# kuboyoo/alphazero-general-ori

Measured on AMD Instinct MI355X. Metric: self-play rollouts/sec (32k boards, 2p Splendor) at 1/2/4/8 MI355X, higher is better.
Workload: dtype fp32 (network) / int8 (boards) / f64 (tree statistics)

## Files before the change

alphazero-general-ori_amd/csrc/mcts.hip:

```cpp
#include <hip/hip_runtime.h>

#include <cmath>
#include <cstring>
#include <new>

#include "../../include/splendor_amd.h"

#include "board_phases.h"
#include "mcts_device.h"
#include "nn_stage.h"
#include "spl_ctx.h"

using namespace spl;

#ifndef SPL_BOUNDS_CHECK
#define SPL_BOUNDS_CHECK 0
#endif
#if SPL_BOUNDS_CHECK
__device__ unsigned long long g_bounds[4 + 64];
__device__ __noinline__ void bounds_note(int site, long long v, int t) {
    atomicAdd(&g_bounds[4 + (site & 63)], 1ull);
    if (atomicAdd(&g_bounds[0], 1ull) == 0) {
        g_bounds[1] = (unsigned long long)v; g_bounds[2] = (unsigned long long)site; g_bounds[3] = (unsigned long long)t;
    }
// ... 504 lines not shown
constexpr int GC_WG_MAX_PROBE = 1024;
__device__ unsigned long long g_gc_probe[GC_WG_MAX_PROBE][16];
__device__ unsigned long long g_gc_probe_max[GC_WG_MAX_PROBE][8];
#define GPROBE(k)                                                                 \
    if (threadIdx.x == 0) {                                                       \
        const uint64_t c_ = __builtin_readcyclecounter();                         \
        gacc[k] += c_ - glast;                                                    \
        glast = c_;                                                               \
    }
#else
#define GPROBE(k)
#endif
constexpr int GC_NOFIT = -2;
#ifndef GC_SR
#define GC_SR 8
#endif
#ifndef GC_CR
#define GC_CR 4
#endif
template <int CR = 4>
__device__ int compact_tree(const Pools &P, int t, int root, int root_round, const GcScr &S, GcLds &L,
                            int bunits, bool linked = false) {
    const int tid = threadIdx.x;
    TreeHdr *H = P.hdr + t;
    const int nc = H->node_count;
    const int rootl = root >= 0 ? node_l(P, root) : -1;
    int32_t *remap = S.remap;
#if GC_PROBE
    uint64_t gacc[8] = {0, 0, 0, 0, 0, 0, 0, 0}, glast = __builtin_readcyclecounter();
    const uint64_t gstart = glast;
#endif
    if (linked) {
        if (tid < 64) mark_linked(P, t, rootl, remap, S.queue);
        __syncthreads();
    }
    int kept = 0;
    for (int base = 0; base < nc; base += GCT) {
        const int i = base + tid;
        bool keep = false;
        if (i < nc) keep = i == rootl || (linked ? remap[i] == 1 : P.nd[node_g(P, t, i)].h.round > root_round);
        int tot;
        const int ex = block_scan(keep ? 1 : 0, tot, L);
        if (i < nc) remap[i] = keep ? kept + ex : -1;
        kept += tot;
    }
    __syncthreads();
    GPROBE(0)
    for (int i = tid; i < nc; i += GCT) {
        int sz = -1;
        if (remap[i] >= 0) {
            sz = 0;
            const int g = node_g(P, t, i);
            const Node nd = P.nd[g];
            if (!nd.h.term) sz = nd.c.ec + REC_UNITS * nd.c.vcnt();
        }
        S.nvs[i] = sz;
    }
    __syncthreads();
    if (tid < 64) {
        const int l = tid;
        int run = 0;
        constexpr int PD = 4;
        int pre[PD];
#pragma unroll
        for (int d = 0; d < PD; d++) pre[d] = 64 * d + l < nc ? S.nvs[64 * d + l] : -1;
        for (int base = 0; base < nc; base += 64) {
            const int i = base + l;
            const int szk = pre[0];
#pragma unroll
            for (int d = 0; d + 1 < PD; d++) pre[d] = pre[d + 1];
            pre[PD - 1] = base + 64 * PD + l < nc ? S.nvs[base + 64 * PD + l] : -1;
            const bool kept = szk >= 0;
            const int sz = kept ? szk : 0;
            bool pending = sz > 0;
            int start = run;
            for (;;) {
                const int x = pending ? sz : 0;
                int incl = x;
#pragma unroll
                for (int o = 1; o < 64; o <<= 1) {
                    const int y = __shfl_up(incl, o, 64);
                    if (l >= o) incl += y;
                }
                const int st = run + incl - x;
                const bool strad = pending && (st & (UPG - 1)) + sz > UPG;
                const uint64_t m = __ballot(strad);
                if (!m) {
                    if (pending) start = st;
                    run += __shfl(incl, 63, 64);
                    break;
                }
                const int f = __ffsll((unsigned long long)m) - 1;
                if (pending && l < f) { start = st; pending = false; }
                run = (__builtin_amdgcn_readlane(st, f) & ~(UPG - 1)) + UPG;
            }
            if (kept) S.nvs[i] = start;
        }
        if (l == 0) L.bc[0] = run;
    }
    __syncthreads();
    const int run = L.bc[0];
    GPROBE(1)
    if (run > H->epg * UPG) return GC_NOFIT;
    __syncthreads();
    int my_units = 0;
    for (int base = 0; base < nc; base += GCT) {
        const int i = base + tid;
        const int ni = i < nc ? remap[i] : -1;
        uint64_t k0 = 0, k1 = 0;
        Node nd{};
        int vs = 0;
        if (ni >= 0) {
            const int g = node_g(P, t, i);
            k0 = P.nkey0[g]; k1 = P.nkey1[g];
            nd = P.nd[g];
            vs = S.nvs[i];
        }
        __syncthreads();
        if (ni >= 0) {
            const int ng = node_g(P, t, ni);
            const bool term = nd.h.term;
            const int ec = nd.c.ec, vcnt = term ? 0 : nd.c.vcnt();
            const int sz = term ? 0 : ec + REC_UNITS * vcnt;
            Node w = nd;
            S.queue[ni] = term ? -1 : nd.h.bchild;
            S.ost[ni] = nd.c.eb(); S.ovb[ni] = nd.c.vb(); S.oec[ni] = term ? 0 : ec;
            if (!term) {
                w.c.set_eb(ec > 0 ? unit_g(P, t, vs) : 0, vcnt);
                w.c.set_vb(vcnt > 0 ? unit_g(P, t, vs + ec) : 0, vcnt);
            }
            w.h.h2 = -1; w.h.h3 = -1;
            P.nkey0[ng] = k0; P.nkey1[ng] = k1;
            P.nd[ng] = w;
            S.cs[ni] = vs; S.cnt[ni] = sz; S.inv[ni] = i;
            my_units += sz;
        }
    }
    int units;
    (void)block_scan(my_units, units, L);
    GPROBE(2)
    for (int ni = tid; ni < kept; ni += GCT) {
        const int ch = S.queue[ni];
        if (ch >= 0) {
            BCHK(IN_TREE(P, t, ch, nc), 56, ((long long)ni << 32) | (uint32_t)ch, t, (void)0);
            const int nl = remap[node_l(P, ch)];
            P.nd[node_g(P, t, ni)].h.bchild = nl >= 0 ? node_g(P, t, nl) : -1;
            BCHK(nl < 0 || P.nd[node_g(P, t, nl)].h.round == P.nd[node_g(P, t, ni)].h.round + 1, 40,
                 ((long long)ni << 32) | (uint32_t)nl, t, (void)0);
        }
    }
    for (int k = tid; k < run; k += GCT) S.own[k] = -1;
    __syncthreads();
    for (int ni = tid; ni < kept; ni += GCT) {
        const int c0 = S.cs[ni], c = S.cnt[ni];
        for (int e = 0; e < c; e++) S.own[c0 + e] = ni;
    }
    __syncthreads();
    GPROBE(3)
    constexpr int SR = GC_SR;
    for (int k0 = 0; k0 < run; k0 += GCT * SR) {
        int j[SR];
#pragma unroll
        for (int r = 0; r < SR; r++) {
            const int k = k0 + GCT * r + tid;
            j[r] = k < run ? S.own[k] : -1;
        }
        int64_t src[SR];
        bool link[SR];
#pragma unroll
        for (int r = 0; r < SR; r++) {
            src[r] = 0; link[r] = false;
            if (j[r] >= 0) {
                const int rel = k0 + GCT * r + tid - S.cs[j[r]], ec = S.oec[j[r]];
                if (rel < ec) {
                    src[r] = S.ost[j[r]] + rel;
                } else {
                    const int rr = rel - ec;
                    src[r] = S.ovb[j[r]] + rr;
                    link[r] = rr % REC_UNITS == REC_LINK_UNIT;
                }
            }
        }
        uint64_t v[SR];
#pragma unroll
        for (int r = 0; r < SR; r++) v[r] = j[r] >= 0 ? P.eu[src[r]] : 0;
#pragma unroll
// ... 470 lines not shown
            for (int k = 0; k < 7; k++) P.out_valid[slot * 7 + k] = P.ex_valid[x * 7 + k];
#pragma unroll
            for (int i = 0; i < 4; i++) {
                const int src = (i + px) % N;
                P.out_winner[slot * 4 + i] = i < N ? r[src < N ? src : 0] : 0.f;
                P.out_scdiff[slot * 4 + i] = i < N ? f[src < N ? src : 0] - f[px < N ? px : 0] : 0;
                P.out_q[slot * 4 + i] = P.ex_q[x * 4 + i];
            }
            P.out_meta[slot * 4 + 0] = (int)gb;
            P.out_meta[slot * 4 + 1] = gno;
            P.out_meta[slot * 4 + 2] = j;
            P.out_meta[slot * 4 + 3] = px;
            P.flq[fq0 + j] = make_int2((int)x, (int)slot);
        }
        __threadfence_block();
        __builtin_amdgcn_wave_barrier();
        if (l == 0) H->games_done += 1;
        deal_game<N>(P, C, t, b, ub[w]);
        nxt = 0;
    } else if (l == 0) {
        H->player = nxt;
        H->episode_step = step;
    }
    __threadfence_block();
    __builtin_amdgcn_wave_barrier();
    wave_store_board<N>(P.board + (size_t)t * Lx::S, b);
    wave_roll_players<N>(s, b, nxt);
    begin_search<N>(P, C, t, s, !ended, false);
    const int nroot = uniform(H->root);
    if (nroot >= 0 && uniform(H->noise_pending) && !uniform(H->gc_queued)) {
        const Node nd0 = P.nd[nroot];
        NodeRun r = run_of(nd0.c);
        r.eb = (int64_t)uniform64((uint64_t)r.eb); r.vb = (int64_t)uniform64((uint64_t)r.vb);
        r.ec = uniform(r.ec);
        const int cand = noise_kept_root(P, C, t, r, ST_DIR | (uint32_t)uniform(H->move_no), pbits[w],
                                         reinterpret_cast<float *>(pterm[w]), pprior[w], pact[w],
                                         reinterpret_cast<int16_t *>(pcnt[w]),
                                         reinterpret_cast<double *>(pprior[w]), (int)(sizeof(pprior[w]) / 8));
        wave_lds_fence();
        int ca;
        float cp, np;
        wave_cand(P, r.eb, r.ec, cand, ca, cp, np);
        const bool forced = uniform(H->forced) != 0;
        Pick pk{-1, 0, -1, 0};
        if (!forced) pk = scan_run(P, r, nd0.h.ns, nd0.h.qs, C.cpuct, C.fpu, false, 0);
        if (l == 0) {
            H->noise_pending = 0;
            Node w2 = nd0;
            w2.c.cand = (int16_t)cand; w2.c.ca = (int16_t)ca; w2.c.cp = cp; w2.c.np = np;
            w2.h.set_pick(pk.e, pk.a, pk.e >= 0 && pk.child >= 0 ? P.nd[pk.child].h.term : 0);
            w2.h.bchild = pk.e >= 0 ? pk.child : -1;
            w2.h.h2 = -1; w2.h.h3 = -1;
            w2.h.bvi = pk.e >= 0 ? P.ep(r.eb + pk.e)->vi : (int16_t)-1;
            P.nd[nroot] = w2;
        }
    }
}

__device__ __forceinline__ void grid_copy(void *dst, const void *src, size_t bytes) {
    const size_t tid = (size_t)blockIdx.x * blockDim.x + threadIdx.x, nth = (size_t)gridDim.x * blockDim.x;
    if (((uintptr_t)dst | (uintptr_t)src) % 16 == 0) {
        const size_t nv = bytes / 16;
        uint4 *d = (uint4 *)dst;
        const uint4 *s = (const uint4 *)src;
        for (size_t i = tid; i < nv; i += nth) d[i] = s[i];
        for (size_t i = nv * 16 + tid; i < bytes; i += nth) ((uint8_t *)dst)[i] = ((const uint8_t *)src)[i];
    } else {
        for (size_t i = tid; i < bytes; i += nth) ((uint8_t *)dst)[i] = ((const uint8_t *)src)[i];
    }
}

__global__ void k_drain_copy(Pools P, int S, int max, int8_t *st, float *pi, uint64_t *valid,
                             float *winner, int32_t *scdiff, float *q, int32_t *meta, int n) {
    const int k = min(P.counters[0], min(max, P.out_cap));
    if (pi) grid_copy(pi, P.out_pi, (size_t)k * SPL_ACTIONS * 4);
    if (st) grid_copy(st, P.out_state, (size_t)k * S);
    if (valid) grid_copy(valid, P.out_valid, (size_t)k * 7 * 8);
    if (meta) grid_copy(meta, P.out_meta, (size_t)k * 4 * 4);
    const size_t tid = (size_t)blockIdx.x * blockDim.x + threadIdx.x, nth = (size_t)gridDim.x * blockDim.x;
    for (size_t i = tid; i < (size_t)k * n; i += nth) {
        const size_t e = i / (size_t)n, j = i - e * (size_t)n;
        if (winner) winner[i] = P.out_winner[e * 4 + j];
        if (scdiff) scdiff[i] = P.out_scdiff[e * 4 + j];
        if (q) q[i] = P.out_q[e * 4 + j];
    }
}

__global__ void k_drain_reset(Pools P, int max, int32_t *n_out) {
    const int c = P.counters[0];
    const int k = min(c, min(max, P.out_cap));
    if (n_out) *n_out = k;
    P.counters[1] += min(c, P.out_cap) - k;
    P.counters[0] = 0;
}

__device__ __forceinline__ void term_values(const Pools &P, int g, float v[4]) {
    const float4 e = *reinterpret_cast<const float4 *>(&P.nd[g].c);
    v[0] = e.x; v[1] = e.y; v[2] = e.z; v[3] = e.w;
}
__device__ __forceinline__ Node term_node(const float v[4], int rd) {
    Node n{};
    n.h.bchild = -1; n.h.h2 = -1; n.h.h3 = -1; n.h.set_pick(-1, 0, 0); n.h.ns = 0;
    n.h.term = 1; n.h.round = (uint8_t)rd; n.h.qs = 0.0;
    *reinterpret_cast<float4 *>(&n.c) = make_float4(v[0], v[1], v[2], v[3]);
    n.h.bvi = -1;
    n.c.ec = 0; n.c.cand = 0; n.c.ca = 0; n.c.pad = 0; n.c.cp = 0.f; n.c.np = -1.f;
    return n;
// ... 27 lines not shown
    uint64_t a = 0, b = 0;
    for (int i = 0; i < Lay<N>::ROWS; i++) {
        const uint64_t x = row(s, i) | ((uint64_t)i << 56);
        a ^= mix64(x ^ 0x243F6A8885A308D3ull);
        b ^= mix64(x ^ 0x13198A2E03707344ull);
    }
    k0 = a;
    k1 = b | 1ull;
}
template <int N>
__device__ __forceinline__ void lane_tree_step(int8_t *s, int a) {
    Chance ch{nullptr, 0, 0, 0, 0};
    int nxt;
    switch (move_kind_of(a)) {
        case MK_GEMS: nxt = make_move<N, MK_GEMS>(s, a, 0, true, ch); break;
        case MK_BUY: nxt = make_move<N, MK_BUY>(s, a, 0, true, ch); break;
        case MK_RESERVE: nxt = make_move<N, MK_RESERVE>(s, a, 0, true, ch); break;
        default: nxt = make_move<N, MK_BUY_RESERVED>(s, a, 0, true, ch); break;
    }
    if (nxt) lane_roll_players<N>(s, nxt);
}

#ifndef SELECT_PROBE
#define SELECT_PROBE 0
#endif
#if SELECT_PROBE
__device__ unsigned long long g_sel_probe[16];
#define SPROBE(k)                                                  \
    {                                                              \
        const uint64_t c_ = __builtin_readcyclecounter();          \
        pacc[k] += c_ - plast;                                     \
        plast = c_;                                                \
    }
#else
#define SPROBE(k)
#endif
#ifndef PATH_CHUNK
#define PATH_CHUNK 8
#endif
enum { LS_DESCEND = 0, LS_EXPAND = 1, LS_DONE = 2 };

#ifndef SELECT_ASM
#define SELECT_ASM 1
#endif
#define SEL_STORES 2
#define SEL_W_OWN 3
#define SEL_W_HINT 8
#define SEL_W_HINT1 9
static_assert(SEL_W_OWN == 1 + SEL_STORES, "own child load: behind SC + the stores");
static_assert(SEL_W_HINT == SEL_STORES + 2 * (1 + SEL_STORES) && SEL_W_HINT1 == SEL_W_HINT + 1,
              "hinted record: two levels back");
#define SEL_STR2(x) #x
#define SEL_STR(x) SEL_STR2(x)
#define SEL_BODY(SA, SC, K)                                                                     \
    "v_cmp_le_i32 vcc, 0, v240\n"                       \
    "v_cmp_le_i32 %[T], 0, v243\n"                      \
    "s_and_b64 vcc, vcc, %[T]\n"                                                               \
    "v_cmp_gt_i32 %[T], %[pcap], v233\n"                \
    "s_and_b64 vcc, vcc, %[T]\n"                                                               \
    "s_and_b64 exec, exec, vcc\n"                                                              \
    "s_cbranch_execz L_done_%=\n"                                                              \
    "v_cmp_ne_u32 vcc, v240, v234\n"                  \
    "s_and_saveexec_b64 %[SV], vcc\n"                   \
    "s_mov_b64 %[INV], exec\n"                                                                 \
    "s_cbranch_execz L_nf" K "_%=\n"                                                           \
    "v_mad_u64_u32 v[238:239], %[CC], v240, 64, %[nd]\n"                                       \
    "global_load_dwordx4 " SA ", v[238:239], off\n"                                            \
    "L_nf" K "_%=:\n"                                                                          \
    "s_mov_b64 exec, %[SV]\n"                                                                  \
    "v_cmp_gt_u32 vcc, %[lim], v242\n"                  \
    "v_cndmask_b32 v226, v240, v242, vcc\n"             \
    "v_mad_u64_u32 v[238:239], %[CC], v226, 64, %[nd]\n"                                       \
    "global_load_dwordx4 " SC ", v[238:239], off\n"                                            \
    "v_mad_u64_u32 v[238:239], %[CC], v233, 4, v[252:253]\n"         \
    "global_store_dword v[238:239], v232, off\n"                                               \
    "v_and_b32 v236, 0xffff, v243\n"                                \
    "v_bfe_u32 v237, v243, 16, 15\n"                                                           \
    "v_lshl_or_b32 v236, v237, 9, v236\n"                                                      \
    "v_mad_u64_u32 v[238:239], %[CC], v233, 4, v[254:255]\n"                                   \
    "global_store_dword v[238:239], v236, off\n"                                               \
    "v_add_u32 v233, 1, v233\n"                                                                \
    "v_mov_b32 v232, v240\n"                                                                   \
    "v_mov_b32 v234, v235\n"                       \
    "v_mov_b32 v235, v226\n"                                                                   \
    "s_cmp_eq_u64 %[INV], 0\n"                                                                 \
    "s_cbranch_scc1 L_av" K "_%=\n"                                                            \
    "s_waitcnt vmcnt(" SEL_STR(SEL_W_OWN) ")\n"          \
    "s_mov_b32 %[F], 1\n"                                                                      \
    "s_branch L_sel" K "_%=\n"                                                                 \
    "L_av" K "_%=:\n"                                   \
    "s_cmp_eq_u32 %[F], 0\n"                            \
    "s_cbranch_scc1 L_a8" K "_%=\n"                     \
    "s_waitcnt vmcnt(" SEL_STR(SEL_W_HINT1) ")\n"                                              \
    "s_branch L_a0" K "_%=\n"                                                                  \
    "L_a8" K "_%=:\n"                                                                          \
    "s_waitcnt vmcnt(" SEL_STR(SEL_W_HINT) ")\n"                                               \
    "L_a0" K "_%=:\n"                                                                          \
    "s_mov_b32 %[F], 0\n"                                                                      \
    "L_sel" K "_%=:\n"
#define SEL_TAKE(R)                                                                             \
    "v_mov_b32 v240, v" #R "\n"                                                                \
    "v_mov_b32 v241, v" #R "+1\n"
__device__ __forceinline__ void descend_linked_asm(int &node, int &depth, NodeLink &rec, const Node *nd, int pcap,
                                                   int32_t *path_n, int32_t *path_x, uint64_t runm, int lim) {
    int r0 = rec.bchild, r1 = rec.h2, r2 = rec.h3;
    int r3 = (int)((uint32_t)(uint16_t)rec.best | ((uint32_t)rec.babt << 16));
    uint64_t T, SV, INV, CC, SAVE;
    int F;
    asm volatile(
        "s_mov_b64 %[SAVE], exec\n"
        "s_mov_b32 %[F], 1\n"
        "v_mov_b32 v232, %[node]\n"
        "v_mov_b32 v233, %[depth]\n"
        "v_mov_b32 v240, %[r0]\n"
        "v_mov_b32 v241, %[r1]\n"
        "v_mov_b32 v242, %[r2]\n"
        "v_mov_b32 v243, %[r3]\n"
        "v_mov_b32 v234, -1\n"
        "v_mov_b32 v235, -1\n"
        "v_mov_b64 v[252:253], %[pn]\n"
        "v_mov_b64 v[254:255], %[pxp]\n"
        "s_and_b64 exec, exec, %[runm]\n"
        "s_cbranch_execz L_done_%=\n"
        "L_top_%=:\n"
        SEL_BODY("v[244:247]", "v[228:231]", "0")
// ... 530 lines not shown
    if (l == 0 && has_c) { bu = uc; ba = ac; bo = rc; }
    for (int base = 0; base < vcnt; base += 64) {
        const int k = base + l;
        if (k < vcnt) {
            const VisitRec v = *P.vr(vb + REC_UNITS * k);
            const int n = k == vidx ? n1 : v.n;
            const double q = k == vidx ? q1 : v.q;
            const double u = ucb_visited(q, n, v.p, cpuct, sq);
            if (u > bu || (u == bu && v.a < ba)) { bu = u; ba = v.a; bo = v.off; bc = v.child; bv = k; }
        }
    }
    const double mu = wave_max_f64(bu);
    const int am = wave_min_i32(bu == mu ? ba : 0x7fffffff);
    const int ln = __ffsll((unsigned long long)__ballot(bu == mu && ba == am)) - 1;
    rank = __builtin_amdgcn_readlane(bo, ln);
    act = am;
    child = __builtin_amdgcn_readlane(bc, ln);
    rvi = __builtin_amdgcn_readlane(bv, ln);
}

struct Level {
    int node, off, act, child;
    int ns;
    double qs;
    NodeRun r;
    int16_t ca;
    uint8_t round;
    float cp, np;
    EdgeP e;
    int n;
    double q;
    int rchild;
    int grow;
    int64_t nb;
};

__device__ __forceinline__ void load_levels_at(const Pools &P, int t, int d, int depth, int lid, Level &V, bool in) {
    const int32_t *path_n = P.path_n + (size_t)t * (P.pcap + 1);
    const int32_t *path_x = P.path_x + (size_t)t * P.pcap;
    V.node = 0; V.off = 0; V.act = 0; V.child = -1; V.ns = 0; V.qs = 0.0;
    V.r = NodeRun{0, 0, 0, 0, 0, 0}; V.e = EdgeP{0.f, 0, -1}; V.n = 0; V.q = Q_UNSET; V.rchild = -1;
    V.grow = 0; V.nb = -1; V.ca = 0; V.round = 0; V.cp = 0.f; V.np = -1.f;
    if (!in) return;
    V.node = path_n[d];
    const int px = path_x[d];
    V.child = d + 1 < depth ? path_n[d + 1] : lid;
    V.off = px_off(px); V.act = px_action(px);
    const Node nd = P.nd[V.node];
    V.ns = nd.h.ns; V.qs = nd.h.qs; V.round = nd.h.round;
    V.r = run_of(nd.c);
    V.ca = nd.c.ca; V.cp = nd.c.cp; V.np = nd.c.np;
    if (nd.h.best == V.off && nd.h.bvi >= 0) V.e = EdgeP{0.f, (int16_t)V.act, nd.h.bvi};
    else V.e = *P.ep(V.r.eb + V.off);
    if (V.e.vi >= 0) {
        const VisitRec v = *P.vr(V.r.vb + REC_UNITS * V.e.vi);
        V.n = v.n; V.q = v.q; V.rchild = v.child;
    } else if (V.r.vcnt == V.r.vcap) {
        V.grow = d == 0 ? (int)V.r.ec : (V.r.vcap == 0 ? 1 : min(2 * (int)V.r.vcap, (int)V.r.ec));
    }
}

__device__ __forceinline__ int grow_at(const Pools &P, int t, int d, bool in) {
    if (!in) return 0;
    const int node = P.path_n[(size_t)t * (P.pcap + 1) + d];
    const int off = px_off(P.path_x[(size_t)t * P.pcap + d]);
    const Node *nd = P.nd + node;
    const int best = nd->h.best, bvi = nd->h.bvi;
    const uint64_t ebq = nd->c.ebq, vbq = nd->c.vbq;
    const int ec = nd->c.ec, vcap = (int)(ebq >> 48), vcnt = (int)(vbq >> 48);
    const int vi = best == off && bvi >= 0 ? bvi : P.ep((int64_t)(ebq & LOW48) + off)->vi;
    if (vi >= 0 || vcnt != vcap) return 0;
    return d == 0 ? ec : (vcap == 0 ? 1 : min(2 * vcap, ec));
}

#ifndef BACKUP_PROBE
#define BACKUP_PROBE 0
#endif
#if BACKUP_PROBE
constexpr int BK_PSLOTS = 32768;
__device__ unsigned long long g_bk_probe[BK_PSLOTS][16];
#define BPROBE(k)                                                  \
    {                                                              \
        const uint64_t c_ = __builtin_readcyclecounter();          \
        bacc[k] += c_ - blast;                                     \
        blast = c_;                                                \
    }
#else
#define BPROBE(k)
#endif

#ifndef WD_MAX
#define WD_MAX 4
#endif
__device__ __forceinline__ int hbase() { return lane_id() & 32; }
__device__ __forceinline__ int half_min_i32(int x) {
#pragma unroll
    for (int o = 16; o > 0; o >>= 1) x = min(x, __shfl_xor(x, o, 64));
    return x;
}
__device__ __forceinline__ int half_sum_i32(int x) {
#pragma unroll
    for (int o = 16; o > 0; o >>= 1) x += __shfl_xor(x, o, 64);
    return x;
}
__device__ __forceinline__ double half_max_f64(double x) {
#pragma unroll
    for (int o = 16; o > 0; o >>= 1) {
        const int lo = __shfl_xor(__double2loint(x), o, 64), hi = __shfl_xor(__double2hiint(x), o, 64);
        x = fmax(x, __hiloint2double(hi, lo));
    }
    return x;
}
__device__ __forceinline__ float half_max_f32(float x) {
#pragma unroll
    for (int o = 16; o > 0; o >>= 1) x = fmaxf(x, __shfl_xor(x, o, 64));
    return x;
}
__device__ __forceinline__ int64_t shfl64(int64_t x, int src) {
    const int lo = __shfl((int)(uint32_t)(uint64_t)x, src, 64), hi = __shfl((int)((uint64_t)x >> 32), src, 64);
    return (int64_t)(((uint64_t)(uint32_t)hi << 32) | (uint32_t)lo);
}
__device__ __forceinline__ float half_np_sum409(const float *a) {
    const int l = lane_id() & 31, hb = hbase();
    const int blk = (l >> 3) & 3, j = l & 7;
    const int off = blk == 0 ? 0 : (blk == 1 ? 96 : (blk == 2 ? 200 : 304));
    const int len = blk == 0 ? 96 : (blk == 3 ? 105 : 104);
    float r = a[off + j];
    for (int i = 8; i < len - (len % 8); i += 8) r += a[off + i + j];
    float r1 = __shfl_xor(r, 1, 64);
    float p01 = (j & 1) ? r1 + r : r + r1;
    float p23 = __shfl_xor(p01, 2, 64);
    float q = (j & 2) ? p23 + p01 : p01 + p23;
    float q2 = __shfl_xor(q, 4, 64);
// ... 176 lines not shown
                if ((wd >> bit) & 1) {
                    const int r = run + __popcll(wd & ((1ull << bit) - 1));
                    S.cp[r] = noise ? pr[64 * k + bit] : pr[64 * k + bit] / psum;
                    S.ca[r] = (int16_t)(64 * k + bit);
                }
            }
            run += __popcll(wd);
        }
        if (hl < 4) S.cp[ec + hl] = -INFINITY;
        wave_lds_only_fence();
        half_write_new_run(P, eb, ec, S.cp, S.ca);
    }
    BPROBE(8)
    {
        int bsel = -1, bact = 0;
        double bu = -INFINITY;
        int ba = 0x7fffffff;
        float pm = -1.f;
        const bool narg = expand && depth > 0;
        if (expand) {
            const double fpu_init = fpu_base(C.fpu, (double)val[0]), sq_eps = sqrt(1e-8);
            for (int i = hl; i < ec; i += 32) {
                const float p = S.cp[i];
                pm = fmaxf(pm, p);
                if (narg) {
                    const double u = ucb_unvisited(p, C.cpuct, fpu_init, sq_eps);
                    if (u > bu || (u == bu && S.ca[i] < ba)) { bu = u; ba = S.ca[i]; }
                }
            }
        }
        const double mu = half_max_f64(bu);
        bact = half_min_i32(bu == mu ? ba : 0x7fffffff);
        pm = half_max_f32(pm);
        int r = 0, cam = 0x7fffffff;
        float npm = -1.f;
        if (expand) {
            const float pb = narg ? S.pr[bact] / psum : 0.f;
            for (int i = hl; i < ec; i += 32) {
                const float p = S.cp[i];
                const int a = S.ca[i];
                r += (p > pb) || (p == pb && a < bact);
                if (p == pm) cam = min(cam, a);
                else npm = fmaxf(npm, p);
            }
        }
        r = half_sum_i32(r);
        cam = half_min_i32(cam);
        npm = half_max_f32(npm);
        if (narg) bsel = r;
        else bact = 0;
        BPROBE(9)
        if (expand && hl == 0) {
            P.nkey0[g] = h_k0; P.nkey1[g] = h_k1;
            Node nn;
            nn.h.bchild = -1; nn.h.h2 = -1; nn.h.h3 = -1;
            nn.h.set_pick(bsel, bact, 0); nn.h.ns = 0;
            nn.h.term = 0; nn.h.round = (uint8_t)h_round; nn.h.bvi = -1;
            nn.h.qs = (double)val[0];
            nn.c.set_eb(eb, 0); nn.c.set_vb(0, 0);
            nn.c.ec = (int16_t)ec; nn.c.cand = 0; nn.c.ca = (int16_t)cam; nn.c.pad = 0;
            nn.c.cp = pm; nn.c.np = pm > 0.f ? npm : -1.f;
            P.nd[g] = nn;
            if (h_hslot >= 0) P.hslot[(size_t)t * P.hcap + h_hslot] = g;
            else hash_insert(P, t, h_k0, g);
            if (depth == 0) H->root = g;
            H->node_count = h_nc + 1;
        }
        if (expand) lid = g;
    }
    const int lidA = __builtin_amdgcn_readlane(lid, 0), lidB = __builtin_amdgcn_readlane(lid, 32);
    const int kindA = __builtin_amdgcn_readlane(kind, 0), kindB = __builtin_amdgcn_readlane(kind, 32);
    const int doneA = __builtin_amdgcn_readlane((int)done, 0), doneB = __builtin_amdgcn_readlane((int)done, 32);
    float valA[4], valB[4];
#pragma unroll
    for (int i = 0; i < 4; i++) {
        valA[i] = __int_as_float(__builtin_amdgcn_readlane(__float_as_int(val[i]), 0));
        valB[i] = __int_as_float(__builtin_amdgcn_readlane(__float_as_int(val[i]), 32));
    }
    if (in0 && !(sel0 ? doneB : doneA) && (sel0 ? kindB : kindA) == LEAF_NN && d0 == (sel0 ? dB : dA) - 1)
        V.child = sel0 ? lidB : lidA;
    BPROBE(1)
    int moved = 0x7fffffff, n_wide_lo = 0, n_wide_hi = 0, n_big_lo = 0, n_big_hi = 0;
    for (int k = 0; k < iters; k++) {
        int sel, d;
        const bool inl = lev(k, sel, d);
        const int tk = sel ? tB : tA, depk = sel ? dB : dA, kk = sel ? kindB : kindA, lk = sel ? lidB : lidA;
        const bool in = !(sel ? doneB : doneA) && inl;
        const uint64_t selm = __ballot(sel);
        if (k > 0) {
            load_levels_at(P, tk, d, depk, lk, V, in);
            if (in && V.grow > 0) V.nb = P.path_b[(size_t)tk * P.pcap + d];
        }
        const bool reloc = in && V.e.vi < 0 && V.grow > 0 && V.nb >= 0 && V.r.vcnt > 0;
        {
            const uint64_t bm = __ballot(reloc && V.grow >= 128);
            n_big_lo += __popcll(bm & ~selm); n_big_hi += __popcll(bm & selm);
        }
        for (uint64_t gm = __ballot(reloc); gm; gm &= gm - 1) {
            const int j = __ffsll((unsigned long long)gm) - 1;
            const int64_t ob = readlane64(V.r.vb, j), nb = readlane64(V.nb, j);
            const int nu = REC_UNITS * __builtin_amdgcn_readlane((int)V.r.vcnt, j);
            for (int k = l; k < nu; k += 64) P.eu[nb + k] = P.eu[ob + k];
        }
        const int64_t ovb = V.r.vb;
        const int ovc = V.r.vcnt;
        int n1 = 0, vidx = -1, nns = 0;
        double q1 = 0.0, nqs = 0.0;
        if (in) {
            const int rot = (depk - d) % N, vi = (N - rot) % N;
            float vr = sel ? valB[0] : valA[0];
#pragma unroll
            for (int i = 1; i < N; i++) vr = vi == i ? (sel ? valB[i] : valA[i]) : vr;
            const double v0 = (double)vr;
            nqs = ((double)(V.ns + 1) * V.qs + v0) / (double)(V.ns + 2);
            nns = V.ns + 1;
            q1 = ((double)V.n * V.q + v0) / (double)(V.n + 1);
            n1 = V.n + 1;
            if (V.e.vi >= 0) {
                vidx = V.e.vi;
                VisitRec *R = P.vr(V.r.vb + REC_UNITS * vidx);
                R->q = q1;
                R->n = n1;
                if (V.rchild < 0 && V.child >= 0) R->child = V.child;
            } else if (V.grow > 0 && V.nb < 0) {
                vidx = -1;
            } else {
                if (V.grow > 0) {
                    V.r.vb = V.nb;
                    V.r.vcap = (int16_t)V.grow;
                }
                vidx = V.r.vcnt;
                *P.vr(V.r.vb + REC_UNITS * vidx) = VisitRec{q1, n1, V.e.p, V.child, (int16_t)V.off, (int16_t)V.act};
                P.ep(V.r.eb + V.off)->vi = (int16_t)vidx;
                V.r.vcnt = (int16_t)(vidx + 1);
                if (V.off == V.r.cand) {
                    int cd, ca;
                    lane_cand(P, V.r.eb, V.r.ec, V.off + 1, cd, ca, V.cp, V.np);
                    V.r.cand = (int16_t)cd; V.ca = (int16_t)ca;
                }
                NodeCold c;
                c.set_eb(V.r.eb, V.r.vcap); c.set_vb(V.r.vb, V.r.vcnt);
                c.ec = (int16_t)V.r.ec; c.cand = (int16_t)V.r.cand; c.ca = (int16_t)V.ca; c.pad = 0;
                c.cp = V.cp; c.np = V.np;
                P.nd[V.node].c = c;
            }
            V.rchild = V.rchild >= 0 ? V.rchild : V.child;
        }
        BPROBE(2)
#if BACKUP_PROBE
        bgroups++;
#endif
        const bool wide = in && V.r.vcnt > BK_WIDE;
        {
            const uint64_t wm = __ballot(wide && d > 0);
            n_wide_lo += __popcll(wm & ~selm); n_wide_hi += __popcll(wm & selm);
        }
        Screen Sc = screen_init(nns, nqs, C.cpuct, C.fpu);
        bool has_c = false;
        double uc = 0.0;
        int ac = 0, rc = 0;
        if (in && V.r.cand < V.r.ec) {
            has_c = true;
            rc = V.r.cand; ac = V.ca;
            screen_item(Sc, false, V.cp, 0, 0.0, rc, V.ca, -1);
            if (V.np >= 0.f) screen_item(Sc, false, V.np, 0, 0.0, 0, 0, -1);
        }
        const int myv = in && !wide ? V.r.vcnt : 0;
        const int maxv = wave_max_i32(myv);
        {
            const int64_t vb0 = myv && ovc ? ovb : 0;
            const auto head = [&](int i) { return *P.vh(vb0 + REC_UNITS * (i < myv && i < ovc ? i : 0)); };
            VisitHead hd[BK_PF];
#pragma unroll
            for (int k = 0; k < BK_PF; k++) hd[k] = head(k);
            for (int base = 0; base < maxv; base += BK_PF) {
#pragma unroll
                for (int k = 0; k < BK_PF; k++) {
                    const int i = base + k;
                    const bool mine = i == vidx;
                    screen_visited(Sc, i < myv, mine && i >= ovc ? V.e.p : hd[k].p, mine ? n1 : hd[k].n,
                                   mine ? q1 : hd[k].q, i);
                    hd[k] = head(base + BK_PF + k);
                }
            }
        }
        if (Sc.vi >= 0) {
            if (Sc.vi == vidx) {
                Sc.off = V.off; Sc.a = V.act; Sc.child = V.rchild;
            } else {
                const VisitTail tl = *P.vt(ovb + REC_UNITS * Sc.vi);
                Sc.off = tl.off; Sc.a = tl.a; Sc.child = tl.child;
            }
        }
        bool open = in && (wide || !(Sc.H2 < Sc.L1));
        int bsel = Sc.off, bact = Sc.a, bch = Sc.child, bvi = Sc.vi;
        if (open && has_c) {
            double u;
            rc = best_unvisited(P, V.r.eb, V.r.ec, V.r.cand, C.cpuct, fpu_base(C.fpu, nqs), sqrt((double)nns + 1e-8),
                                u, ac);
            uc = u;
        }
        if (__ballot(open)) wave_lds_fence();
        BPROBE(3)
// ... 360 lines not shown
    if (hipMemcpyFromSymbol(out16, HIP_SYMBOL(g_sel_probe), 16 * 8) != hipSuccess) return SPL_EDEVICE;
    if (reset) {
        unsigned long long z[16] = {0};
        if (hipMemcpyToSymbol(HIP_SYMBOL(g_sel_probe), z, sizeof(z)) != hipSuccess) return SPL_EDEVICE;
    }
    return 0;
}
#endif

#if GC_PROBE
int spl_diag_gc_probe(unsigned long long *out24, int reset) {
    static unsigned long long h[GC_WG_MAX_PROBE][16], hm[GC_WG_MAX_PROBE][8];
    if (hipMemcpyFromSymbol(h, HIP_SYMBOL(g_gc_probe), sizeof(h)) != hipSuccess) return SPL_EDEVICE;
    if (hipMemcpyFromSymbol(hm, HIP_SYMBOL(g_gc_probe_max), sizeof(hm)) != hipSuccess) return SPL_EDEVICE;
    for (int k = 0; k < 24; k++) out24[k] = 0;
    for (int i = 0; i < GC_WG_MAX_PROBE; i++) {
        for (int k = 0; k < 10; k++) out24[k] += h[i][k];
        if (h[i][10] > out24[10]) {
            for (int k = 10; k < 14; k++) out24[k] = h[i][k];
            for (int k = 0; k < 7; k++) out24[16 + k] = hm[i][k];
        }
    }
    if (reset) {
        memset(h, 0, sizeof(h));
        memset(hm, 0, sizeof(hm));
        if (hipMemcpyToSymbol(HIP_SYMBOL(g_gc_probe), h, sizeof(h)) != hipSuccess) return SPL_EDEVICE;
        if (hipMemcpyToSymbol(HIP_SYMBOL(g_gc_probe_max), hm, sizeof(hm)) != hipSuccess) return SPL_EDEVICE;
    }
    return 0;
}
#endif

#if LM_PROBE
int spl_diag_lm_probe(unsigned long long *out) {
    return hipMemcpyFromSymbol(out, HIP_SYMBOL(g_lm_probe), sizeof(g_lm_probe)) == hipSuccess ? 0 : SPL_EDEVICE;
}
#endif

#if BACKUP_PROBE
int spl_diag_backup_probe(unsigned long long *out16, int reset) {
    static unsigned long long h[BK_PSLOTS][16];
    if (hipMemcpyFromSymbol(h, HIP_SYMBOL(g_bk_probe), sizeof(h)) != hipSuccess) return SPL_EDEVICE;
    for (int k = 0; k < 16; k++) out16[k] = 0;
    for (int i = 0; i < BK_PSLOTS; i++)
        for (int k = 0; k < 16; k++) out16[k] += h[i][k];
    if (reset) {
        memset(h, 0, sizeof(h));
        if (hipMemcpyToSymbol(HIP_SYMBOL(g_bk_probe), h, sizeof(h)) != hipSuccess) return SPL_EDEVICE;
    }
    return 0;
}
#endif

#if SPL_BOUNDS_CHECK
int spl_diag_bounds(unsigned long long *out4, int reset) {
    if (hipMemcpyFromSymbol(out4, HIP_SYMBOL(g_bounds), 68 * 8) != hipSuccess) return SPL_EDEVICE;
    if (reset) {
        unsigned long long z[68] = {0};
        if (hipMemcpyToSymbol(HIP_SYMBOL(g_bounds), z, sizeof(z)) != hipSuccess) return SPL_EDEVICE;
    }
    return 0;
}
#endif

long long spl_mcts_plan_bytes(const spl_ctx *ctx, int B, const spl_mcts_config *cfg) {
    if (!valid_cfg(ctx, B, cfg)) return SPL_EINVAL;
    return (long long)plan_pools(ctx->n, B, cfg).bytes;
}

int spl_mcts_create(const spl_ctx *ctx, int B, const spl_mcts_config *cfg, spl_mcts **out) {
    if (!valid_cfg(ctx, B, cfg) || !out) return SPL_EINVAL;
    spl_mcts *m = new (std::nothrow) spl_mcts;
    if (!m) return SPL_EINVAL;
    m->n = ctx->n; m->B = B; m->S = 7 * (32 + 10 * ctx->n + ctx->n * ctx->n);
    m->token_limit = ctx->token_limit;
    m->rules = ctx->rules;
    SearchCfg &C = m->cfg;
    C.cpuct = cfg->cpuct; C.fpu = cfg->fpu; C.dir_alpha = cfg->dirichlet_alpha;
    C.dir_temp = cfg->dirichlet_temp > 0 ? cfg->dirichlet_temp : 1.0;
    C.prob_full = cfg->prob_full; C.num_sims = cfg->num_sims; C.ratio_full = cfg->ratio_full;
    C.forced_playouts = cfg->forced_playouts; C.dirichlet = cfg->dirichlet_alpha > 0;
    C.temp_threshold = cfg->temp_threshold; C.seed = cfg->seed; C.board_base = cfg->board_base;
    C.selfplay = cfg->selfplay;
    C.edge_reserve = 48;
    Pools &P = m->P;
    const Plan L = plan_pools(ctx->n, B, cfg);
    P.nmax = L.nmax; P.emax = L.emax; P.hcap = L.hcap; P.pcap = L.pcap;
    P.nptab = L.nptab; P.eptab = L.eptab;
    P.npages = (int)L.npages; P.epages = (int)L.epages;
    P.ntrees = B;
    P.nhome = min(min(SPL_HOME_N, P.nptab), (int)(L.npages / (4 * (long long)B)));
    while (P.nhome & (P.nhome - 1)) P.nhome &= P.nhome - 1;
    P.ehome = min(min(SPL_HOME_E, P.eptab), (int)(L.epages / (4 * (long long)B)));
    const size_t nn = (size_t)L.npages * NPG, ne = (size_t)L.epages * UPG;
    const int excap = L.excap;
    const size_t nx = (size_t)B * excap, no = (size_t)L.out_cap;
    const int gcw = B < GC_WG ? B : GC_WG;
    void *arena = nullptr;
    if (hipMalloc(&arena, L.bytes) != hipSuccess) { delete m; return SPL_EDEVICE; }
    m->arena = arena;
    m->bytes = L.bytes;
    char *p = (char *)arena;
    P.hdr = carve<TreeHdr>(p, B);
    P.nkey0 = carve<uint64_t>(p, nn); P.nkey1 = carve<uint64_t>(p, nn);
    P.nd = carve<Node>(p, nn);
    P.eu = carve<uint64_t>(p, ne);
    P.ntab = carve<int32_t>(p, (size_t)B * P.nptab); P.etab = carve<int32_t>(p, (size_t)B * P.eptab);
    P.npidx = carve<int32_t>(p, (size_t)P.npages); P.epidx = carve<int32_t>(p, (size_t)P.epages);
    P.nfree = carve<int32_t>(p, (size_t)P.npages); P.efree = carve<int32_t>(p, (size_t)P.epages);
    P.alloc = carve<int32_t>(p, 16);
    P.hslot = carve<int32_t>(p, (size_t)B * P.hcap);
    P.path_n = carve<int32_t>(p, (size_t)B * (P.pcap + 1));
    P.path_x = carve<int32_t>(p, (size_t)B * P.pcap);
    P.path_b = carve<int64_t>(p, (size_t)B * P.pcap);
    P.gc_stride = gc_ints(P.nmax, P.emax);
    P.gscr = carve<int32_t>(p, (size_t)gcw * P.gc_stride);
    P.root_state = carve<int8_t>(p, (size_t)B * m->S);
    P.excap = excap; P.out_cap = (int)no;
    P.board = carve<int8_t>(p, (size_t)B * m->S);
    P.ex_state = carve<int8_t>(p, nx * m->S); P.ex_pi = carve<float>(p, nx * SPL_ACTIONS);
    P.ex_q = carve<float>(p, 4 * nx); P.ex_valid = carve<uint64_t>(p, 7 * nx);
    P.ex_player = carve<int32_t>(p, nx);
    P.out_state = carve<int8_t>(p, no * m->S); P.out_pi = carve<float>(p, no * SPL_ACTIONS);
    P.out_winner = carve<float>(p, 4 * no); P.out_q = carve<float>(p, 4 * no);
    P.out_valid = carve<uint64_t>(p, 7 * no); P.out_scdiff = carve<int32_t>(p, 4 * no);
    P.out_meta = carve<int32_t>(p, 4 * no); P.counters = carve<int32_t>(p, 16);
    P.nbrd = L.nbb ? carve<int8_t>(p, (size_t)L.nbb * nn) : nullptr;
    P.gcq = carve<int32_t>(p, (size_t)B);
    P.gcq2 = carve<int32_t>(p, (size_t)B);
    P.flq = carve<int2>(p, no);
    bool ok = hipMemset(P.hdr, 0, sizeof(TreeHdr) * B) == hipSuccess &&
              hipMemset(P.counters, 0, 64) == hipSuccess &&
              hipMemset(P.hslot, 0xFF, 4 * (size_t)B * P.hcap) == hipSuccess;
    if (ok) {
        hipLaunchKernelGGL(k_init_pools, dim3(1024), dim3(256), 0, (hipStream_t)0, P, B);
        ok = hipGetLastError() == hipSuccess && hipDeviceSynchronize() == hipSuccess;
    }
    if (!ok) { (void)hipFree(arena); delete m; return SPL_EDEVICE; }
    *out = m;
    return 0;
}

int spl_mcts_destroy(spl_mcts *m) {
    if (!m) return 0;
    (void)hipFree(m->arena);
    delete m;
    return 0;
}

long long spl_mcts_device_bytes(const spl_mcts *m) {
    if (!m) return SPL_EINVAL;
    return (long long)m->bytes;
}

int spl_mcts_rules(const spl_mcts *m) { return m ? m->rules : SPL_EINVAL; }

int spl_mcts_set_roots(spl_mcts *m, const int8_t *roots, int keep_tree, int force_full, void *hs) {
    return spl_mcts_set_roots_active(m, roots, nullptr, keep_tree, force_full, hs);
}
// ... 214 lines not shown
```

alphazero-general-ori_amd/csrc/mcts_device.h:

```cpp
#pragma once
#include "splendor_device.h"

namespace spl {

constexpr double Q_UNSET = -42.0;

struct TreeHdr {
    int32_t node_count, edge_count, root, sims_done;
    int32_t budget, full, noise_pending, depth;
    int32_t leaf_kind, player, episode_step, move_no;
    int32_t game_no, overflow, n_examples, leaf_round;
    uint64_t leaf_k0, leaf_k1;
    float leaf_v[4];
    int32_t games_done, forced, moves, wd_search;
    int32_t prunes, resets, unexpanded, gc_state;
    int64_t units_gc;
    int64_t enext;
    int32_t npg, epg, eleft, live_gc;
    int32_t root_round, gc_queued, withdrawals, gcs;
    int32_t leaf_hslot, leaf_slot;
    int32_t depth_max, depth_sum;
    int32_t resume;
    int32_t sims_backed, exact_wide, big_moves;
};
static_assert(sizeof(TreeHdr) == 208, "TreeHdr layout (splendor/mcts.py HDR_DTYPE)");
enum { LEAF_NONE = 0, LEAF_NN = 1, LEAF_TERMINAL = 2 };

struct EdgeP {
    float p;
    int16_t a;
    int16_t vi;
};
static_assert(sizeof(EdgeP) == 8, "EdgeP layout");
struct VisitRec {
    double q;
    int32_t n;
    float p;
    int32_t child;
    int16_t off;
    int16_t a;
};
static_assert(sizeof(VisitRec) == 24, "VisitRec layout");
constexpr int REC_UNITS = 3;
constexpr int REC_LINK_UNIT = 2;
struct VisitHead {
    double q;
    int32_t n;
    float p;
};
struct VisitTail {
    int32_t child;
    int16_t off;
    int16_t a;
};

struct NodeHot {
    int32_t bchild;
    int32_t h2, h3;
    int16_t best;
    uint16_t babt;
    int32_t ns;
    uint8_t term;
    uint8_t round;
    int16_t bvi;
    double qs;
    __device__ __forceinline__ int ba() const { return babt & 0x7FFF; }
    __device__ __forceinline__ int bterm() const { return babt >> 15; }
    __device__ __forceinline__ void set_pick(int rank, int a, int term_child) {
        best = (int16_t)rank;
        babt = (uint16_t)(a | (term_child << 15));
    }
};
struct __align__(16) NodeLink {
    int32_t bchild, h2, h3;
    int16_t best;
    uint16_t babt;
    __device__ __forceinline__ int ba() const { return babt & 0x7FFF; }
    __device__ __forceinline__ int bterm() const { return babt >> 15; }
};
constexpr uint64_t LOW48 = (1ull << 48) - 1;
struct NodeCold {
    uint64_t ebq;
    uint64_t vbq;
    int16_t ec;
    int16_t cand;
    int16_t ca;
    int16_t pad;
    float cp;
    float np;
    __device__ __forceinline__ int64_t eb() const { return (int64_t)(ebq & LOW48); }
    __device__ __forceinline__ int64_t vb() const { return (int64_t)(vbq & LOW48); }
    __device__ __forceinline__ int vcap() const { return (int)(ebq >> 48); }
    __device__ __forceinline__ int vcnt() const { return (int)(vbq >> 48); }
    __device__ __forceinline__ void set_eb(int64_t eb, int vcap) { ebq = (uint64_t)eb | ((uint64_t)vcap << 48); }
    __device__ __forceinline__ void set_vb(int64_t vb, int vcnt) { vbq = (uint64_t)vb | ((uint64_t)vcnt << 48); }
};
struct __align__(64) Node {
    NodeHot h;
    NodeCold c;
};
static_assert(sizeof(NodeHot) == 32 && sizeof(NodeCold) == 32 && sizeof(Node) == 64 && sizeof(NodeLink) == 16,
              "Node layout");
__device__ __forceinline__ NodeLink link_of(const Node *nd, int g) {
    return *reinterpret_cast<const NodeLink *>(&nd[g].h);
}

struct NodeRun {
    int64_t eb, vb;
    int16_t ec, vcnt, vcap, cand;
};
__device__ __forceinline__ NodeRun run_of(const NodeCold &c) {
    return NodeRun{c.eb(), c.vb(), c.ec, (int16_t)c.vcnt(), (int16_t)c.vcap(), c.cand};
}

constexpr int NPG_SHIFT = 6, NPG = 1 << NPG_SHIFT;
constexpr int UPG_SHIFT = 11, UPG = 1 << UPG_SHIFT;
static_assert(UPG >= 4 * 409, "a node's allocation fits one edge page");

struct Pools {
    int nmax, emax, hcap, pcap;
    int nptab, eptab;
    int npages, epages;
    int ntrees;
    int nhome, ehome;
    TreeHdr *hdr;
    uint64_t *nkey0, *nkey1;
    Node *nd;
    uint64_t *eu;
    int32_t *ntab, *etab;
    int32_t *npidx, *epidx;
    int32_t *nfree, *efree;
    int32_t *alloc;
    int32_t *hslot;
    int32_t *path_n;
    int32_t *path_x;
    int64_t *path_b;
    int32_t *gscr;
    size_t gc_stride;
    int8_t *nbrd;
    int8_t *root_state;
    int excap, out_cap;
    int8_t *board;
    int8_t *ex_state;
    float *ex_pi, *ex_q;
    uint64_t *ex_valid;
    int32_t *ex_player;
    int8_t *out_state;
    float *out_pi, *out_winner, *out_q;
    uint64_t *out_valid;
    int32_t *out_scdiff, *out_meta;
    int32_t *counters;
    int32_t *gcq;
    int32_t *gcq2;
    int2 *flq;

    __device__ __forceinline__ EdgeP *ep(int64_t u) const { return reinterpret_cast<EdgeP *>(eu + u); }
    __device__ __forceinline__ VisitRec *vr(int64_t u) const { return reinterpret_cast<VisitRec *>(eu + u); }
    __device__ __forceinline__ const VisitHead *vh(int64_t u) const { return reinterpret_cast<const VisitHead *>(eu + u); }
    __device__ __forceinline__ const VisitTail *vt(int64_t u) const {
        return reinterpret_cast<const VisitTail *>(eu + u + REC_LINK_UNIT);
    }
};

__device__ __forceinline__ int node_g(const Pools &P, int t, int i) {
    const int pi = i >> NPG_SHIFT;
    const int pg = pi < P.nhome ? t * P.nhome + pi : P.ntab[(size_t)t * P.nptab + pi];
    return pg * NPG + (i & (NPG - 1));
}
__device__ __forceinline__ int node_l(const Pools &P, int g) {
    const int pg = g >> NPG_SHIFT;
    const int pi = pg < P.nhome * P.ntrees ? (pg & (P.nhome - 1)) : P.npidx[pg];
    return pi * NPG + (g & (NPG - 1));
}
__device__ __forceinline__ int64_t unit_g(const Pools &P, int t, int v) {
    const int pi = v >> UPG_SHIFT;
    const int64_t pg = pi < P.ehome ? (int64_t)t * P.ehome + pi : (int64_t)P.etab[(size_t)t * P.eptab + pi];
    return pg * UPG + (v & (UPG - 1));
}

template <int N>
struct NodeBoard {
    static constexpr int BYTES = (Lay<N>::LS + 15) & ~15;
    static constexpr int UNITS = BYTES / 16;
};

struct SearchCfg {
    double cpuct, fpu, dir_alpha, dir_temp, prob_full;
    int num_sims, ratio_full, forced_playouts, dirichlet;
    int temp_threshold, selfplay;
    int edge_reserve;
    uint64_t seed;
    uint32_t board_base;
};

enum : uint32_t { ST_FULL = 1u << 24, ST_DIR = 2u << 24, ST_PICK = 3u << 24, ST_MOVE = 4u << 24,
                  ST_DEAL = 5u << 24, ST_BEST = 6u << 24,
                  ST_PLAYER = 8u << 24 };

__device__ __forceinline__ uint64_t wave_xor64(uint64_t x) {
#pragma unroll
    for (int o = 32; o > 0; o >>= 1) x ^= __shfl_xor(x, o, 64);
    return x;
}

__device__ __forceinline__ void wave_argmax(double &u, int &i) {
#pragma unroll
    for (int o = 32; o > 0; o >>= 1) {
        double u2 = __shfl_xor(u, o, 64);
        int i2 = __shfl_xor(i, o, 64);
        if (u2 > u || (u2 == u && i2 < i)) { u = u2; i = i2; }
    }
}

template <int CTRL>
__device__ __forceinline__ double dpp_f64(double v) {
    const int lo = __double2loint(v), hi = __double2hiint(v);
// ... 206 lines not shown
```

Before: 76.08 million.

## Inline first two visit records into a 128-byte MCTS node

Node grows from 64 to 128 bytes and now holds up to two visit records inline, addressed through the edge-unit pool via a computed base offset. Nodes with few visits no longer allocate or chase separate visit-record storage, and GC compaction relinks the inline children. Select asm stride, allocation sizing and arena layout change to match. It doubles node memory and bandwidth per node load, which the hot descend path pays.

```diff
diff --git a/alphazero-general-ori_amd/csrc/mcts.hip b/alphazero-general-ori_amd/csrc/mcts.hip
--- a/alphazero-general-ori_amd/csrc/mcts.hip
+++ b/alphazero-general-ori_amd/csrc/mcts.hip
@@ -580,7 +580,8 @@
             sz = 0;
             const int g = node_g(P, t, i);
             const Node nd = P.nd[g];
-            if (!nd.h.term) sz = nd.c.ec + REC_UNITS * nd.c.vcnt();
+            const int vcnt = nd.c.vcnt();
+            if (!nd.h.term) sz = nd.c.ec + (vcnt > NODE_INLINE_RECS ? REC_UNITS * vcnt : 0);
         }
         S.nvs[i] = sz;
     }
@@ -636,30 +637,50 @@
         const int i = base + tid;
         const int ni = i < nc ? remap[i] : -1;
         uint64_t k0 = 0, k1 = 0;
-        Node nd{};
+        u32x4 rq[7] = {};
         int vs = 0;
         if (ni >= 0) {
             const int g = node_g(P, t, i);
             k0 = P.nkey0[g]; k1 = P.nkey1[g];
-            nd = P.nd[g];
+            const u32x4 *src = reinterpret_cast<const u32x4 *>(P.nd + g);
+#pragma unroll
+            for (int k = 0; k < 7; k++) rq[k] = src[k];
             vs = S.nvs[i];
         }
         __syncthreads();
         if (ni >= 0) {
             const int ng = node_g(P, t, ni);
+            Node nd;
+            static_assert(offsetof(Node, rsv) == 7 * sizeof(u32x4), "the moved part of a record");
+            __builtin_memcpy(&nd, rq, sizeof(rq));
             const bool term = nd.h.term;
             const int ec = nd.c.ec, vcnt = term ? 0 : nd.c.vcnt();
-            const int sz = term ? 0 : ec + REC_UNITS * vcnt;
+            const bool inl = vcnt <= NODE_INLINE_RECS;
+            const int sz = term ? 0 : ec + (inl ? 0 : REC_UNITS * vcnt);
             Node w = nd;
             S.queue[ni] = term ? -1 : nd.h.bchild;
             S.ost[ni] = nd.c.eb(); S.ovb[ni] = nd.c.vb(); S.oec[ni] = term ? 0 : ec;
             if (!term) {
-                w.c.set_eb(ec > 0 ? unit_g(P, t, vs) : 0, vcnt);
-                w.c.set_vb(vcnt > 0 ? unit_g(P, t, vs + ec) : 0, vcnt);
+                w.c.set_eb(ec > 0 ? unit_g(P, t, vs) : 0, inl ? NODE_INLINE_RECS : vcnt);
+                w.c.set_vb(inl ? inline_vb(P, ng) : unit_g(P, t, vs + ec), vcnt);
+                const auto relink = [&](uint64_t u, bool live) -> uint64_t {
+                    const int ch = (int)(uint32_t)u;
+                    if (!live || ch < 0) return u;
+                    BCHK(IN_TREE(P, t, ch, nc), 57, ((long long)ni << 32) | (uint32_t)ch, t, (void)0);
+                    const int nl = remap[node_l(P, ch)];
+                    const int nch = nl >= 0 ? node_g(P, t, nl) : -1;
+                    return (u & 0xFFFFFFFF00000000ull) | (uint64_t)(uint32_t)nch;
+                };
+                static_assert(NODE_INLINE_RECS == 2, "the inline records' links, one by one");
+                w.inl[REC_LINK_UNIT] = relink(nd.inl[REC_LINK_UNIT], inl && vcnt > 0);
+                w.inl[REC_UNITS + REC_LINK_UNIT] = relink(nd.inl[REC_UNITS + REC_LINK_UNIT], inl && vcnt > 1);
             }
             w.h.h2 = -1; w.h.h3 = -1;
             P.nkey0[ng] = k0; P.nkey1[ng] = k1;
-            P.nd[ng] = w;
+            __builtin_memcpy(rq, &w, sizeof(rq));
+            u32x4 *dst = reinterpret_cast<u32x4 *>(P.nd + ng);
+#pragma unroll
+            for (int k = 0; k < 7; k++) dst[k] = rq[k];
             S.cs[ni] = vs; S.cnt[ni] = sz; S.inv[ni] = i;
             my_units += sz;
         }
@@ -1236,7 +1257,8 @@
             w2.h.bchild = pk.e >= 0 ? pk.child : -1;
             w2.h.h2 = -1; w2.h.h3 = -1;
             w2.h.bvi = pk.e >= 0 ? P.ep(r.eb + pk.e)->vi : (int16_t)-1;
-            P.nd[nroot] = w2;
+            P.nd[nroot].h = w2.h;
+            P.nd[nroot].c = w2.c;
         }
     }
 }
@@ -1370,6 +1392,8 @@
               "hinted record: two levels back");
 #define SEL_STR2(x) #x
 #define SEL_STR(x) SEL_STR2(x)
+#define SEL_NODE_SHL 1
+static_assert(sizeof(Node) == (size_t)64 << SEL_NODE_SHL, "descend_linked_asm: the record stride");
 #define SEL_BODY(SA, SC, K)                                                                     \
     "v_cmp_le_i32 vcc, 0, v240\n"                       \
     "v_cmp_le_i32 %[T], 0, v243\n"                      \
@@ -1382,13 +1406,15 @@
     "s_and_saveexec_b64 %[SV], vcc\n"                   \
     "s_mov_b64 %[INV], exec\n"                                                                 \
     "s_cbranch_execz L_nf" K "_%=\n"                                                           \
-    "v_mad_u64_u32 v[238:239], %[CC], v240, 64, %[nd]\n"                                       \
+    "v_lshlrev_b32 v227, " SEL_STR(SEL_NODE_SHL) ", v240\n"                                    \
+    "v_mad_u64_u32 v[238:239], %[CC], v227, 64, %[nd]\n"                                       \
     "global_load_dwordx4 " SA ", v[238:239], off\n"                                            \
     "L_nf" K "_%=:\n"                                                                          \
     "s_mov_b64 exec, %[SV]\n"                                                                  \
     "v_cmp_gt_u32 vcc, %[lim], v242\n"                  \
     "v_cndmask_b32 v226, v240, v242, vcc\n"             \
-    "v_mad_u64_u32 v[238:239], %[CC], v226, 64, %[nd]\n"                                       \
+    "v_lshlrev_b32 v227, " SEL_STR(SEL_NODE_SHL) ", v226\n"                                    \
+    "v_mad_u64_u32 v[238:239], %[CC], v227, 64, %[nd]\n"                                       \
     "global_load_dwordx4 " SC ", v[238:239], off\n"                                            \
     "v_mad_u64_u32 v[238:239], %[CC], v233, 4, v[252:253]\n"         \
     "global_store_dword v[238:239], v232, off\n"                                               \
@@ -2025,7 +2051,13 @@
     V.ca = nd.c.ca; V.cp = nd.c.cp; V.np = nd.c.np;
     if (nd.h.best == V.off && nd.h.bvi >= 0) V.e = EdgeP{0.f, (int16_t)V.act, nd.h.bvi};
     else V.e = *P.ep(V.r.eb + V.off);
-    if (V.e.vi >= 0) {
+    if (V.e.vi >= 0 && V.r.vcnt <= NODE_INLINE_RECS) {
+        const bool hi = V.e.vi > 0;
+        static_assert(NODE_INLINE_RECS == 2, "the record picked by one select");
+        const uint64_t u0 = hi ? nd.inl[REC_UNITS] : nd.inl[0], u1 = hi ? nd.inl[REC_UNITS + 1] : nd.inl[1];
+        const uint64_t u2 = hi ? nd.inl[REC_UNITS + 2] : nd.inl[2];
+        V.q = __longlong_as_double((long long)u0); V.n = (int)(uint32_t)u1; V.rchild = (int)(uint32_t)u2;
+    } else if (V.e.vi >= 0) {
         const VisitRec v = *P.vr(V.r.vb + REC_UNITS * V.e.vi);
         V.n = v.n; V.q = v.q; V.rchild = v.child;
     } else if (V.r.vcnt == V.r.vcap) {
@@ -2052,6 +2084,7 @@
 #if BACKUP_PROBE
 constexpr int BK_PSLOTS = 32768;
 __device__ unsigned long long g_bk_probe[BK_PSLOTS][16];
+__device__ unsigned long long g_bk_hist[2][5];
 #define BPROBE(k)                                                  \
     {                                                              \
         const uint64_t c_ = __builtin_readcyclecounter();          \
@@ -2334,12 +2367,12 @@
         BPROBE(9)
         if (expand && hl == 0) {
             P.nkey0[g] = h_k0; P.nkey1[g] = h_k1;
-            Node nn;
+            Node nn{};
             nn.h.bchild = -1; nn.h.h2 = -1; nn.h.h3 = -1;
             nn.h.set_pick(bsel, bact, 0); nn.h.ns = 0;
             nn.h.term = 0; nn.h.round = (uint8_t)h_round; nn.h.bvi = -1;
             nn.h.qs = (double)val[0];
-            nn.c.set_eb(eb, 0); nn.c.set_vb(0, 0);
+            nn.c.set_eb(eb, NODE_INLINE_RECS); nn.c.set_vb(inline_vb(P, g), 0);
             nn.c.ec = (int16_t)ec; nn.c.cand = 0; nn.c.ca = (int16_t)cam; nn.c.pad = 0;
             nn.c.cp = pm; nn.c.np = pm > 0.f ? npm : -1.f;
             P.nd[g] = nn;
@@ -2431,6 +2464,7 @@
         BPROBE(2)
 #if BACKUP_PROBE
         bgroups++;
+        if (in && vidx >= 0) atomicAdd(&g_bk_hist[d == 0 ? 0 : 1][min((int)V.r.vcnt, 5) - 1], 1ull);
 #endif
         const bool wide = in && V.r.vcnt > BK_WIDE;
         {
@@ -2897,6 +2931,17 @@
 }
 #endif
 
+#if BACKUP_PROBE
+int spl_diag_backup_hist(unsigned long long *out10, int reset) {
+    if (hipMemcpyFromSymbol(out10, HIP_SYMBOL(g_bk_hist), 10 * 8) != hipSuccess) return SPL_EDEVICE;
+    if (reset) {
+        unsigned long long z[10] = {0};
+        if (hipMemcpyToSymbol(HIP_SYMBOL(g_bk_hist), z, sizeof(z)) != hipSuccess) return SPL_EDEVICE;
+    }
+    return 0;
+}
+#endif
+
 #if SPL_BOUNDS_CHECK
 int spl_diag_bounds(unsigned long long *out4, int reset) {
     if (hipMemcpyFromSymbol(out4, HIP_SYMBOL(g_bounds), 68 * 8) != hipSuccess) return SPL_EDEVICE;
@@ -2948,8 +2993,15 @@
     char *p = (char *)arena;
     P.hdr = carve<TreeHdr>(p, B);
     P.nkey0 = carve<uint64_t>(p, nn); P.nkey1 = carve<uint64_t>(p, nn);
+    P.eu = carve<uint64_t>(p, ne);
     P.nd = carve<Node>(p, nn);
-    P.eu = carve<uint64_t>(p, ne);
+    P.nd_unit_base = (int64_t)(((char *)P.nd - (char *)P.eu) / 8);
+    if ((uintptr_t)P.nd % alignof(Node) != 0 ||
+        P.nd_unit_base + (int64_t)NODE_UNITS * (int64_t)nn >= (int64_t)1 << 48) {
+        (void)hipFree(arena);
+        delete m;
+        return SPL_EINVAL;
+    }
     P.ntab = carve<int32_t>(p, (size_t)B * P.nptab); P.etab = carve<int32_t>(p, (size_t)B * P.eptab);
     P.npidx = carve<int32_t>(p, (size_t)P.npages); P.epidx = carve<int32_t>(p, (size_t)P.epages);
     P.nfree = carve<int32_t>(p, (size_t)P.npages); P.efree = carve<int32_t>(p, (size_t)P.epages);
diff --git a/alphazero-general-ori_amd/csrc/mcts_device.h b/alphazero-general-ori_amd/csrc/mcts_device.h
--- a/alphazero-general-ori_amd/csrc/mcts_device.h
+++ b/alphazero-general-ori_amd/csrc/mcts_device.h
@@ -1,4 +1,6 @@
 #pragma once
+#include <cstddef>
+
 #include "splendor_device.h"
 
 namespace spl {
@@ -95,11 +97,16 @@
     __device__ __forceinline__ void set_eb(int64_t eb, int vcap) { ebq = (uint64_t)eb | ((uint64_t)vcap << 48); }
     __device__ __forceinline__ void set_vb(int64_t vb, int vcnt) { vbq = (uint64_t)vb | ((uint64_t)vcnt << 48); }
 };
-struct __align__(64) Node {
+constexpr int NODE_INLINE_RECS = 2;
+struct __align__(128) Node {
     NodeHot h;
     NodeCold c;
-};
-static_assert(sizeof(NodeHot) == 32 && sizeof(NodeCold) == 32 && sizeof(Node) == 64 && sizeof(NodeLink) == 16,
+    uint64_t inl[NODE_INLINE_RECS * REC_UNITS];
+    uint64_t rsv[2];
+};
+constexpr int NODE_UNITS = 16, NODE_INL_UNIT = 8;
+static_assert(sizeof(NodeHot) == 32 && sizeof(NodeCold) == 32 && sizeof(Node) == 128 && sizeof(NodeLink) == 16 &&
+              sizeof(Node) == 8 * NODE_UNITS && offsetof(Node, inl) == 8 * NODE_INL_UNIT && alignof(Node) == 128,
               "Node layout");
 __device__ __forceinline__ NodeLink link_of(const Node *nd, int g) {
     return *reinterpret_cast<const NodeLink *>(&nd[g].h);
@@ -127,6 +134,7 @@
     uint64_t *nkey0, *nkey1;
     Node *nd;
     uint64_t *eu;
+    int64_t nd_unit_base;
     int32_t *ntab, *etab;
     int32_t *npidx, *epidx;
     int32_t *nfree, *efree;
@@ -162,6 +170,10 @@
     }
 };
 
+__device__ __forceinline__ int64_t inline_vb(const Pools &P, int g) {
+    return P.nd_unit_base + (int64_t)g * NODE_UNITS + NODE_INL_UNIT;
+}
+
 __device__ __forceinline__ int node_g(const Pools &P, int t, int i) {
     const int pi = i >> NPG_SHIFT;
     const int pg = pi < P.nhome ? t * P.nhome + pi : P.ntab[(size_t)t * P.nptab + pi];
```

After: 76.51 million, median of 6. About the same (+0.6%).
